# andrewcharlesjones/spatial-alignment

Hardware: AMD Instinct MI355X
Metric: training steps/sec (ELBO fwd+bwd), 2-view N=10k M=200, 1/2/4/8 GPU (higher is better)
Workload: dtype f32 (fp64 warp layer, covariance whitening and M x M factorisations)

## Files before the change

### include/gpsa_hip.h

```cpp
#ifndef GPSA_HIP_H
#define GPSA_HIP_H

#ifdef __cplusplus
extern "C" {
#endif

enum {
  GPSA_F32 = 0,
  GPSA_F64 = 1,
  GPSA_F32_X64 = 2,
  GPSA_F32_OUT64 = 3,
  GPSA_F32_ACC64 = 4
};
enum { GPSA_K_RBF = 0, GPSA_K_MATERN12 = 1, GPSA_K_MATERN32 = 2 };
enum { GPSA_EINVAL = -1, GPSA_EWORKSPACE = -2, GPSA_EUNSUPPORTED = -3 };

int gpsa_version(void);
const char* gpsa_build_arch(void);
const char* gpsa_source_hash(void);

int gpsa_kmat(int dtype, int in_dtype, int kind, const void* Z, int M, const void* X, long long C,
              int D, const void* ls_u, const void* var_u, double jitter, void* K, void* stream);

long long gpsa_kmat_bwd_workspace(int dtype, int M, long long C, int D);
// ... 65 lines not shown
                              const float* meanT, const double* q, const float* var_u, const float* eps, const float* Y,
                              long long N, int S, const float* noise_u, float* g, float* dmeanT, float* abar, double* part,
                              float* FT, void* workspace, long long workspace_bytes, void* stream);
int gpsa_quadform_elbo_delta_x3_f32(int omega_dtype, const float* alpha, const void* Omega, int M, long long C, int L,
                                    const float* delta, const double* q, const float* var_u, const float* eps,
                                    const float* Y, long long N, int S, const float* noise_u, float* g, float* dmeanT,
                                    float* abar, double* part, float* FT, void* workspace, long long workspace_bytes,
                                    void* stream);
int gpsa_quadform_elbo_skip_f32(int omega_dtype, const float* alpha, const void* Omega, int M, long long C, int L,
                                const float* meanT, const double* q, const float* var_u, const float* eps, const float* Y,
                                long long N, int S, const float* noise_u, float* g, float* dmeanT, float* abar,
                                double* part, float* FT, void* workspace, long long workspace_bytes, void* stream);
int gpsa_quadform_elbo_delta_skip_f32(int omega_dtype, const float* alpha, const void* Omega, int M, long long C, int L,
                                      const float* delta, const double* q, const float* var_u, const float* eps,
                                      const float* Y, long long N, int S, const float* noise_u, float* g, float* dmeanT,
                                      float* abar, double* part, float* FT, void* workspace, long long workspace_bytes,
                                      void* stream);
int gpsa_quadform_bwd_omega(int dtype, int out_dtype, const void* alpha, const void* g, int M, long long C,
                            int L, void* dOmega, void* workspace, long long workspace_bytes, void* stream);
int gpsa_quadform_bwd_omega_takes_delta(int M, long long C);
int gpsa_quadform_bwd_omega_delta_f32(int out_dtype, const float* alpha, const float* g, const float* dmeanT, int M,
                                      long long C, int L, void* dOmega, float* ddelta, double dbeta, void* workspace,
                                      long long workspace_bytes, void* stream);
long long gpsa_quadform_bwd_omega_x3_workspace(int M, long long C, int L);
int gpsa_quadform_bwd_omega_x3(int dtype, int out_dtype, const void* alpha, const void* g, int M, long long C, int L,
                               void* dOmega, void* workspace, long long workspace_bytes, void* stream);
int gpsa_quadform_bwd_omega_delta_x3(int out_dtype, const float* alpha, const float* g, const float* dmeanT, int M,
                                     long long C, int L, void* dOmega, float* ddelta, double dbeta, void* workspace,
                                     long long workspace_bytes, void* stream);

long long gpsa_whiten_workspace(int M);
int gpsa_whiten_f64(const double* Kinv, int in_dtype, const void* Kuf, int M, long long C,
                    int alpha_dtype, void* alpha, double* q, void* workspace, long long workspace_bytes,
                    void* stream);

int gpsa_panel_mm(int dtype, int p_dtype, int transP, const void* P, const void* X, int M, long long C,
                  void* Y, void* colsq, void* workspace, long long workspace_bytes, void* stream);

int gpsa_col_axpy(int dtype, const void* Y, const void* X, const void* d, double s, int M,
                  long long C, void* out, void* stream);

int gpsa_data_sample_fwd(const float* meanT, const float* v, const double* q, const float* var_u,
                         const float* eps, long long C, int L, float* F, float* Sigma, void* stream);
int gpsa_data_sample_bwd(const float* dF, const float* eps, const float* Sigma, const float* var_u,
                         long long C, int L, float* g, float* dmeanT, float* qbar, int dvar_dtype, void* dvar_u,
                         void* workspace, long long workspace_bytes, void* stream);
// ... 507 lines not shown
```

### spatial_alignment_amd/_lib.py

```python
import ctypes as C
import os

_HERE = os.path.dirname(os.path.abspath(__file__))
LIB_PATH = os.path.join(_HERE, "libgpsa_hip.so")

_vp, _i, _ll, _d = C.c_void_p, C.c_int, C.c_longlong, C.c_double

SIGNATURES = {
    "gpsa_version": (_i, []),
    "gpsa_build_arch": (C.c_char_p, []),
    "gpsa_source_hash": (C.c_char_p, []),
    "gpsa_kmat": (_i, [_i, _i, _i, _vp, _i, _vp, _ll, _i, _vp, _vp, _d, _vp, _vp]),
    "gpsa_kmat_bwd_workspace": (_ll, [_i, _i, _ll, _i]),
    "gpsa_kmat_bwd": (_i, [_i, _i, _i, _vp, _i, _vp, _ll, _i, _vp, _vp, _vp, _i, _vp, _vp, _vp, _vp, _ll, _vp]),
    "gpsa_gemm_workspace": (_ll, [_i, _i, _i, _i, _i]),
    "gpsa_gemm": (_i, [_i, _i, _i, _i, _i, _ll, _d, _vp, _ll, _ll, _vp, _ll, _ll, _d, _vp, _ll, _ll,
                       _i, _i, _vp, _ll, _vp]),
    "gpsa_omega_fwd": (_i, [_vp, _i, _i, _d, _vp, _vp]),
    "gpsa_omega_bwd": (_i, [_vp, _vp, _i, _i, _i, _vp, _vp]),
    "gpsa_omega_fwd2": (_i, [_vp, _i, _vp, _vp, _i, _vp, _i, _d, _vp]),
    "gpsa_omega_bwd2": (_i, [_vp, _vp, _vp, _i, _vp, _vp, _vp, _i, _i, _i, _vp]),
    "gpsa_chol_f64": (_i, [_vp, _i, _i, _vp, _vp, _vp]),
    "gpsa_tri_inv_f64": (_i, [_vp, _vp, _i, _i, _vp]),
    "gpsa_chol_inv_f64": (_i, [_vp, _vp, _i, _i, _vp, _vp, _vp]),
    "gpsa_experiment_split_bf16_product": (_i, [_vp, _vp, _i, _ll, _i, _i, _vp, _vp]),
    "gpsa_experiment_split_bf16_rate": (_i, [_i, _i, _vp, _vp]),
    "gpsa_chol_inv_sel_f64": (_i, [_vp, _vp, _i, _i, _i, _i, _i, _vp, _vp, _vp]),
    "gpsa_chol_inv_blocked_workspace": (_ll, [_i, _i]),
    "gpsa_chol_inv_blocked_f64": (_i, [_vp, _vp, _i, _i, _vp, _vp, _vp, _ll, _vp]),
    "gpsa_quadform_workspace": (_ll, [_i, _i, _ll, _i]),
    "gpsa_quadform_fwd": (_i, [_i, _i, _vp, _vp, _i, _ll, _i, _vp, _vp, _ll, _vp]),
    "gpsa_quadform_bwd_alpha": (_i, [_i, _i, _vp, _vp, _vp, _i, _ll, _i, _vp, _vp, _ll, _vp]),
    "gpsa_quadform_fwd_keep": (_i, [_i, _vp, _vp, _i, _ll, _i, _vp, _vp, _vp, _vp, _vp]),
    "gpsa_quadform_bwd_alpha_kept": (_i, [_i, _vp, _vp, _i, _ll, _i, _vp, _vp, _vp, _vp]),
    "gpsa_quadform_bwd_omega": (_i, [_i, _i, _vp, _vp, _i, _ll, _i, _vp, _vp, _ll, _vp]),
    "gpsa_quadform_bwd_omega_takes_delta": (_i, [_i, _ll]),
    "gpsa_quadform_bwd_omega_delta_f32": (_i, [_i, _vp, _vp, _vp, _i, _ll, _i, _vp, _vp, _d, _vp, _ll, _vp]),
    "gpsa_quadform_bwd_omega_x3_workspace": (_ll, [_i, _ll, _i]),
    "gpsa_quadform_bwd_omega_x3": (_i, [_i, _i, _vp, _vp, _i, _ll, _i, _vp, _vp, _ll, _vp]),
    "gpsa_quadform_bwd_omega_delta_x3": (_i, [_i, _vp, _vp, _vp, _i, _ll, _i, _vp, _vp, _d, _vp, _ll, _vp]),
    "gpsa_whiten_workspace": (_ll, [_i]),
    "gpsa_whiten_f64": (_i, [_vp, _i, _vp, _i, _ll, _i, _vp, _vp, _vp, _ll, _vp]),
    "gpsa_panel_mm": (_i, [_i, _i, _i, _vp, _vp, _i, _ll, _vp, _vp, _vp, _ll, _vp]),
    "gpsa_col_axpy": (_i, [_i, _vp, _vp, _vp, _d, _i, _ll, _vp, _vp]),
    "gpsa_data_sample_fwd": (_i, [_vp, _vp, _vp, _vp, _vp, _ll, _i, _vp, _vp, _vp]),
    "gpsa_data_sample_bwd": (_i, [_vp, _vp, _vp, _vp, _ll, _i, _vp, _vp, _vp, _i, _vp, _vp, _ll, _vp]),
    "gpsa_warp_sample_fwd": (_i, [_vp, _vp, _vp, _vp, _vp, _vp, _vp, _vp, _ll, _i, _i, _vp, _vp, _vp, _vp, _vp]),
    "gpsa_warp_sample_bwd": (_i, [_vp, _vp, _vp, _vp, _vp, _vp, _ll, _i, _i, _vp, _vp, _vp, _vp, _vp, _vp, _vp,
                                  _ll, _vp]),
    "gpsa_mean_resid_fwd": (_i, [_vp, _vp, _vp, _vp, _i, _i, _d, _vp, _vp, _vp]),
    "gpsa_mean_resid_bwd": (_i, [_vp, _vp, _vp, _i, _i, _d, _vp, _vp, _vp, _vp, _vp]),
    "gpsa_loglik_fwd": (_i, [_vp, _vp, _vp, _i, _ll, _i, _vp, _vp, _ll, _vp]),
    "gpsa_loglik_bwd": (_i, [_vp, _vp, _vp, _vp, _i, _ll, _i, _vp, _vp, _vp, _ll, _vp]),
    "gpsa_bdot": (_i, [_i, _vp, _ll, _vp, _ll, _ll, _i, _vp, _vp, _ll, _vp]),
    "gpsa_add_diag": (_i, [_i, _vp, _i, _i, _d, _vp]),
    "gpsa_mvn_kl_fwd": (_i, [_vp, _vp, _vp, _ll, _vp, _ll, _vp, _vp, _i, _i, _vp, _vp]),
    "gpsa_mvn_kl_bwd": (_i, [_vp, _vp, _vp, _ll, _vp, _ll, _vp, _vp, _vp, _i, _i, _vp, _vp, _vp, _vp]),
    "gpsa_mvn_kl_grouped_fwd": (_i, [_vp, _vp, _vp, _vp, _vp, _vp, _i, _i, _vp, _vp, _vp]),
    "gpsa_mvn_kl_grouped_bwd": (_i, [_vp, _vp, _vp, _vp, _vp, _vp, _vp, _vp, _vp, _i, _i, _i, _vp, _vp, _vp,
# ... 325 lines not shown
```

### spatial_alignment_amd/csrc/qf_common.hpp

```cpp
#pragma once
#include <stdlib.h>

#include "common.hpp"

namespace gpsa {

typedef float f32x4_t __attribute__((ext_vector_type(4)));

typedef float f32x4 __attribute__((ext_vector_type(4)));
typedef float f32x2 __attribute__((ext_vector_type(2)));

enum { MODE_QUAD = 0, MODE_ACCUM = 1, MODE_STORE = 2 };

enum { PACK_SYM_UPPER = 1, PACK_KSTEP = 2, PACK_KSTEP_LAST = 4 };

typedef __attribute__((address_space(3))) void* lds_ptr_t;

__device__ __forceinline__ void glds16(const float* gsrc, unsigned lds_base) {
  unsigned keep;
  asm volatile(
      "s_mov_b32 %0, m0\n\ts_mov_b32 m0, %2\n\ts_nop 0\n\tglobal_load_lds_dwordx4 %1, off\n\ts_mov_b32 m0, %0"
      : "=&s"(keep)
      : "v"(gsrc), "s"(lds_base)
      : "memory");
// ... 330 lines not shown
    for (int r = MB - 1; r >= 0; --r) {
      int best = -1;
      for (int w = 0; w < 4 && best < 0; ++w)
        if (cnt[w] + r + 1 <= cap) best = w;
      if (best < 0) {
        best = 0;
        for (int w = 1; w < 4; ++w)
          if (cnt[w] < cnt[best]) best = w;
      }
      for (int c = 0; c <= r; ++c) {
        rr[best][cnt[best]] = r;
        cc[best][cnt[best]] = c;
        ++cnt[best];
      }
    }
  }
  constexpr int max_cnt() const {
    int m = 0;
    for (int w = 0; w < 4; ++w) m = cnt[w] > m ? cnt[w] : m;
    return m;
  }
};

#define GPSA_GRAM_SHAPES(X) X(2, 2) X(4, 2) X(7, 2) X(13, 2) X(2, 1) X(4, 1) X(7, 1) X(13, 1) X(16, 1)
#define GPSA_GRAM_EXTERN(MB, NL)                                                \
  extern template __global__ void gram_mfma_kernel<MB, true, NL> GPSA_GRAM_SIG; \
  extern template __global__ void gram_mfma_kernel<MB, false, NL> GPSA_GRAM_SIG;
#define GPSA_GRAM_DEFINE(MB, NL)                                         \
  template __global__ void gram_mfma_kernel<MB, true, NL> GPSA_GRAM_SIG; \
  template __global__ void gram_mfma_kernel<MB, false, NL> GPSA_GRAM_SIG;
GPSA_GRAM_SHAPES(GPSA_GRAM_EXTERN)
constexpr int gram_max_nl(int mb) {
  GPSA_GRAM_SHAPES(GPSA_SHAPE_SECOND)
  return 0;
}
template <typename TO>
__global__ void gram_reduce_kernel(const float* __restrict__ part, int M, int MP, int L, int nsplit, TO* __restrict__ out,
                                   float* __restrict__ ddelta, float dbeta);
extern template __global__ void gram_reduce_kernel<float>(const float* __restrict__, int, int, int, int, float* __restrict__, float* __restrict__, float);
extern template __global__ void gram_reduce_kernel<double>(const float* __restrict__, int, int, int, int, double* __restrict__, float* __restrict__, float);

template <int MB>
__global__ void __launch_bounds__(256, 1) gram_x3_kernel(const unsigned short* __restrict__ img, const float* __restrict__ g,
                                                         const float* __restrict__ dmean, int M, long long C, int L,
                                                         int nsplit, float* __restrict__ part);
#define GPSA_GRAM_X3_SHAPES(X) X(2) X(4) X(7) X(13) X(16)
// ... 9 lines not shown
```

### spatial_alignment_amd/csrc/qf_gram.hip

```cpp
#include "qf_common.hpp"

namespace gpsa {

__device__ __attribute__((aligned(16))) const float gram_zero16[4] = {0.f, 0.f, 0.f, 0.f};


constexpr int GR_G = 4;

template <int MB, int NKB, int W, int NS, int NL, typename STG>
__device__ __forceinline__ void gram_wave_chunk(const float* __restrict__ img,
                                                const float* __restrict__ gvec, int kq,
                                                f32x4 (&acc)[NL][NS + GR_G], STG&& stage, int drow, int lane15) {
  constexpr GramPlan<MB> P{};
  constexpr int N = P.cnt[W];
  constexpr int NGRP = (((NS + GR_G - 1) / GR_G) + 1) & ~1;
  constexpr int NPW_ = (MB * NKB + 3) / 4;
  static_assert(NKB == 4, "one K block per staging wave");
  auto frag = [&](int kb, int tile_row) {
    return *reinterpret_cast<const float4*>(img + kb * (NPW_ * 256) + tile_row * 256);
  };
  auto tile_of = [](int s) { return s < N ? s : N - 1; };
  auto new_row = [&](int s) { return s < N && (s == 0 || P.rr[W][s] != P.rr[W][s - 1]); };
  float4 araw[2][GR_G], fb[2][GR_G];
  float4 gk[NL], gn[NL], arow[NL];
#pragma unroll
  for (int q = 0; q < NL; ++q) {
    gn[q] = gk[q] = *reinterpret_cast<const float4*>(gvec + q * GR_KC + kq * 4);
    arow[q] = make_float4(0.f, 0.f, 0.f, 0.f);
  }
  constexpr bool OWNS_LAST = [] {
    constexpr GramPlan<MB> Q{};
    for (int s = 0; s < Q.cnt[W]; ++s)
      if (Q.rr[W][s] == MB - 1) return true;
    return false;
  }();
  const bool dsel = OWNS_LAST && drow >= 0 && lane15 == drow;
  float4 dk[OWNS_LAST ? NL : 1], dn[OWNS_LAST ? NL : 1];
  if (OWNS_LAST) {
#pragma unroll
    for (int q = 0; q < NL; ++q)
      dn[q] = dk[q] = drow >= 0 ? *reinterpret_cast<const float4*>(gvec + (NL + q) * GR_KC + kq * 4)
                                : make_float4(0.f, 0.f, 0.f, 0.f);
  }
#define GPSA_GR_FETCH(SLOT, KB, GP)                                                           \
  _Pragma("unroll") for (int u = 0; u < GR_G; ++u) {                                          \
    const int t__ = tile_of(GR_G * (GP) + u);                                                 \
    if (new_row(GR_G * (GP) + u)) araw[SLOT][u] = frag(KB, P.rr[W][t__]);                     \
    fb[SLOT][u] = frag(KB, P.cc[W][t__]);                                                     \
  }
  GPSA_GR_FETCH(0, 0, 0)
#pragma unroll 1
  for (int kb = 0; kb < NKB; ++kb) {
#pragma unroll
    for (int q = 0; q < NL; ++q) gk[q] = gn[q];
    if (OWNS_LAST) {
#pragma unroll
      for (int q = 0; q < NL; ++q) dk[q] = dn[q];
    }
#pragma unroll
    for (int gp = 0; gp < NGRP; ++gp) {
      const int cur = gp & 1, nxt = cur ^ 1;
      if (gp + 1 < NGRP) {
        GPSA_GR_FETCH(nxt, kb, gp + 1)
      } else if (kb + 1 < NKB) {
#pragma unroll
        for (int q = 0; q < NL; ++q)
          gn[q] = *reinterpret_cast<const float4*>(gvec + q * GR_KC + (kb + 1) * 16 + kq * 4);
        if (OWNS_LAST && drow >= 0) {
#pragma unroll
          for (int q = 0; q < NL; ++q)
            dn[q] = *reinterpret_cast<const float4*>(gvec + (NL + q) * GR_KC + (kb + 1) * 16 + kq * 4);
        }
        GPSA_GR_FETCH(nxt, kb + 1, 0)
      }
      __builtin_amdgcn_sched_barrier(0);
      if (gp < 5) stage(kb, gp);
      __builtin_amdgcn_sched_barrier(0);
      float4 a[NL][GR_G];
      int sl[GR_G];
#pragma unroll
      for (int u = 0; u < GR_G; ++u) {
        const int s_ = GR_G * gp + u;
        sl[u] = s_ < N ? s_ : NS + u;
#pragma unroll
        for (int q = 0; q < NL; ++q) {
          if (new_row(s_)) {
            const float4 r_ = araw[cur][u];
            arow[q] = make_float4(r_.x * gk[q].x, r_.y * gk[q].y, r_.z * gk[q].z, r_.w * gk[q].w);
            if (OWNS_LAST && P.rr[W][s_ < N ? s_ : N - 1] == MB - 1 && drow >= 0) {
              const float4 d_ = dk[q];
              arow[q] = make_float4(dsel ? d_.x : arow[q].x, dsel ? d_.y : arow[q].y, dsel ? d_.z : arow[q].z,
                                    dsel ? d_.w : arow[q].w);
            }
          }
          a[q][u] = arow[q];
        }
      }
#define GPSA_GR_MMA(F)                                                                          \
  _Pragma("unroll") for (int q = 0; q < NL; ++q)                                                \
    _Pragma("unroll") for (int u = 0; u < GR_G; ++u)                                            \
      if (GR_G * gp + u < N)                                                                    \
        acc[q][sl[u]] = __builtin_amdgcn_mfma_f32_16x16x4f32(a[q][u].F, fb[cur][u].F, acc[q][sl[u]], 0, 0, 0);
      GPSA_GR_MMA(x)
      GPSA_GR_MMA(y)
      GPSA_GR_MMA(z)
      GPSA_GR_MMA(w)
#undef GPSA_GR_MMA
      __builtin_amdgcn_sched_barrier(0);
    }
  }
#undef GPSA_GR_FETCH
}

template <int MB, int W, int NS>
__device__ __forceinline__ void gram_wave_store(const f32x4 (&acc)[NS + GR_G], float* __restrict__ P_, int j,
                                                int kq) {
  constexpr GramPlan<MB> P{};
  constexpr int MP = MB * 16;
#pragma unroll
  for (int s = 0; s < P.cnt[W]; ++s)
#pragma unroll
    for (int r = 0; r < 4; ++r)
      P_[(long long)(P.rr[W][s] * 16 + kq * 4 + r) * MP + P.cc[W][s] * 16 + j] = acc[s][r];
}

template <int MB, bool ALIGNED, int NL, int W>
__device__ __forceinline__ void gram_wave_run(const float* __restrict__ alpha, const float* __restrict__ g,
                                              long long gstride, int M, long long C, int L, int nsplit, float* __restrict__ part,
                                              float* __restrict__ sA_, float* __restrict__ sG_,
                                              const float* __restrict__ dmean) {
  constexpr int MP = MB * 16;
  constexpr GramPlan<MB> PLAN{};
  constexpr int NS = PLAN.max_cnt();
  constexpr int NKB = GR_KC / 16, NPIECE = MB * NKB;
  constexpr int NPW = (NPIECE + 3) / 4;
  constexpr int SA_STRIDE = NPW * 4 * 256, SG_STRIDE = 2 * NL * GR_KC;
  const int nstage = (dmean != nullptr ? 2 : 1) * NL * (GR_KC / 4);
  const int drow = dmean != nullptr ? M - 16 * (MB - 1) : -1;
  const int tid = threadIdx.x, lane = tid & 63;
  constexpr int w = W;
  const int j = lane & 15, kq = lane >> 4;
  const int l0 = blockIdx.x * NL, sp = blockIdx.y;
  const long long nch = (C + GR_KC - 1) / GR_KC;
  const long long ch0 = (long long)sp * nch / nsplit, ch1 = (long long)(sp + 1) * nch / nsplit;

  f32x4 acc[NL][NS + GR_G];
#pragma unroll
  for (int q = 0; q < NL; ++q)
#pragma unroll
    for (int s = 0; s < NS + GR_G; ++s) acc[q][s] = (f32x4){0.f, 0.f, 0.f, 0.f};

  auto gsrc = [&](int ln, long long col) -> const float* {
    const int which = ln / (NL * (GR_KC / 4)), lq = min(l0 + (ln / (GR_KC / 4)) % NL, L - 1);
    if (which == 1) return col >= C ? gram_zero16 : dmean + (long long)lq * C + col;
    return (gstride == C && col >= C) ? gram_zero16 : g + (long long)lq * gstride + col;
  };
#define GPSA_GR_STAGE(CH, BUF)                                                               \
  {                                                                                          \
    const long long cb__ = (long long)(CH) * GR_KC;                                          \
    if (ALIGNED) {                                                                           \
       \
      long long col = cb__ + w * 16 + kq * 4;                                                \
      col = col < C - 4 ? col : C - 4;                                                       \
      _Pragma("unroll") for (int pc = 0; pc < NPW; ++pc) {                                   \
        if ((pc & 3) == 0)                                                                   \
          dma_set_m0(__builtin_amdgcn_readfirstlane(lds_addr(sA_ + (BUF) * SA_STRIDE + (w * NPW + pc) * 256))); \
        int row = (pc < MB ? pc : 0) * 16 + j;                                               \
        row = row < M ? row : M - 1;                                                         \
        const float* gp__ = alpha + (long long)row * C + col;                                \
        if ((pc & 3) == 0) glds16_m0<0>(gp__);                                               \
        if ((pc & 3) == 1) glds16_m0<1024>(gp__ - 256);                                      \
        if ((pc & 3) == 2) glds16_m0<2048>(gp__ - 512);                                      \
        if ((pc & 3) == 3) glds16_m0<3072>(gp__ - 768);                                      \
      }                                                                                      \
      if (lane < nstage) {                                                                   \
        dma_set_m0(__builtin_amdgcn_readfirstlane(lds_addr(sG_ + (BUF) * SG_STRIDE)));       \
        glds16_m0<0>(gsrc(lane, cb__ + (lane % (GR_KC / 4)) * 4));                           \
      }                                                                                      \
    } else {                                                                                 \
      for (int e = tid; e < NPIECE * 256; e += 256) {                                        \
        const int piece = e >> 8, ln = (e >> 2) & 63, r = e & 3;                             \
        const int rb = piece / NKB, kb = piece % NKB;                                        \
        const int row = rb * 16 + (ln & 15);                                                 \
        const long long col = cb__ + kb * 16 + (ln >> 4) * 4 + r;                            \
        sA_[(BUF) * SA_STRIDE + (kb * NPW + rb) * 256 + (e & 255)] =                         \
            (row < M && col < C) ? alpha[(long long)row * C + col] : 0.f;                    \
      }                                                                                      \
      if (tid < NL * GR_KC)           \
        sG_[(BUF) * SG_STRIDE + tid] = g[(long long)min(l0 + tid / GR_KC, L - 1) * gstride + cb__ + tid % GR_KC]; \
    }                                                                                        \
  }

  if (ch1 > ch0) GPSA_GR_STAGE(ch0, 0)
  GPSA_DMA_DRAIN();
  __syncthreads();
  int buf = 0;
  for (long long ch = ch0; ch < ch1; ++ch) {
    const bool more = ch + 1 < ch1;
    constexpr int NGRP_ = (((NS + GR_G - 1) / GR_G) + 1) & ~1;
    constexpr bool SPREAD = ALIGNED && NGRP_ >= 5;
    if (more && !SPREAD) GPSA_GR_STAGE(ch + 1, buf ^ 1)
    const float* img = sA_ + buf * SA_STRIDE + lane * 4;
    long long ncol = (ch + 1) * GR_KC + w * 16 + kq * 4;
    ncol = ncol < C - 4 ? ncol : C - 4;
    const float* nsrc = alpha + ncol;
    float* nimg = sA_ + (buf ^ 1) * SA_STRIDE + w * NPW * 256;
    auto stage = [&](int kb, int gp) {
      if (!SPREAD || !more) return;
      if (gp < 4) {
        const int pc = kb * 4 + gp;
        if (pc < NPW) {
          if (gp == 0) dma_set_m0(__builtin_amdgcn_readfirstlane(lds_addr(nimg + kb * 4 * 256)));
          int row = pc * 16 + j;
          row = row < M ? row : M - 1;
          const float* gp__ = nsrc + (long long)row * C;
          if (gp == 0) glds16_m0<0>(gp__);
          if (gp == 1) glds16_m0<1024>(gp__ - 256);
          if (gp == 2) glds16_m0<2048>(gp__ - 512);
          if (gp == 3) glds16_m0<3072>(gp__ - 768);
        }
      } else if (kb == 0 && lane < nstage) {
        dma_set_m0(__builtin_amdgcn_readfirstlane(lds_addr(sG_ + (buf ^ 1) * SG_STRIDE)));
        glds16_m0<0>(gsrc(lane, (ch + 1) * GR_KC + (lane % (GR_KC / 4)) * 4));
      }
    };
    static_assert(NPW <= 16, "four pieces per K block of the chunk being multiplied");
    gram_wave_chunk<MB, NKB, W, NS, NL>(img, sG_ + buf * SG_STRIDE, kq, acc, stage, drow, lane & 15);
    GPSA_DMA_DRAIN();
    __syncthreads();
    buf ^= 1;
  }
  GPSA_DMA_DRAIN();
#undef GPSA_GR_STAGE
#pragma unroll
  for (int q = 0; q < NL; ++q) {
    if (l0 + q >= L) break;
    float* P = part + ((long long)(l0 + q) * nsplit + sp) * MP * MP;
    gram_wave_store<MB, W, NS>(acc[q], P, j, kq);
  }
}

template <int MB, bool ALIGNED, int NL>
__global__ void __launch_bounds__(256, (MB >= 13 || NL > 1) ? 1 : 2)
gram_mfma_kernel(const float* __restrict__ alpha, const float* __restrict__ g, long long gstride, int M,
                 long long C, int L, int nsplit, float* __restrict__ part, const float* __restrict__ dmean) {
  constexpr int NKB = GR_KC / 16, NPIECE = MB * NKB;
  constexpr int NPW = (NPIECE + 3) / 4;
  __shared__ __attribute__((aligned(16))) float sA[2][NPW * 4 * 256];
  __shared__ __attribute__((aligned(16))) float sG[2][2 * NL * GR_KC];
  const int w = __builtin_amdgcn_readfirstlane(threadIdx.x >> 6);
  switch (w) {
    case 0: gram_wave_run<MB, ALIGNED, NL, 0>(alpha, g, gstride, M, C, L, nsplit, part, &sA[0][0], &sG[0][0], dmean); break;
    case 1: gram_wave_run<MB, ALIGNED, NL, 1>(alpha, g, gstride, M, C, L, nsplit, part, &sA[0][0], &sG[0][0], dmean); break;
    case 2: gram_wave_run<MB, ALIGNED, NL, 2>(alpha, g, gstride, M, C, L, nsplit, part, &sA[0][0], &sG[0][0], dmean); break;
    default: gram_wave_run<MB, ALIGNED, NL, 3>(alpha, g, gstride, M, C, L, nsplit, part, &sA[0][0], &sG[0][0], dmean); break;
  }
}

template <typename TO>
__global__ void gram_reduce_kernel(const float* __restrict__ part, int M, int MP, int L, int nsplit,
                                   TO* __restrict__ out, float* __restrict__ ddelta, float dbeta) {
  const int jj = blockIdx.x * 32 + (threadIdx.x & 31);
  const int i = blockIdx.y * 8 + (threadIdx.x >> 5);
  const int l = blockIdx.z;
  if (ddelta != nullptr && i == M && jj < M) {
    const float* p = part + (long long)l * nsplit * MP * MP + (long long)M * MP + jj;
    const long long mm = (long long)MP * MP;
    double s = 0.0;
    for (int sp = 0; sp < nsplit; ++sp) s += (double)p[sp * mm];
    float* d = ddelta + (long long)jj * L + l;
    *d = dbeta != 0.f ? dbeta * *d + (float)s : (float)s;
    return;
  }
  if (i >= M || jj > i) return;
  const float* p = part + (long long)l * nsplit * MP * MP + (long long)i * MP + jj;
  const long long mm = (long long)MP * MP;
  TO s = TO(0), s1 = TO(0), s2 = TO(0), s3 = TO(0);
  int sp = 0;
  for (; sp + 3 < nsplit; sp += 4) {
    s += (TO)p[sp * mm];
// ... 18 lines not shown
```

### spatial_alignment_amd/csrc/quadform.hip

```cpp
#include <stdlib.h>

#include "qf_common.hpp"

namespace gpsa {

template <typename T>
int gemm_launch(int transA, int transB, int m, int n, long long k, double alpha, const T* A,
                long long lda, long long sA, const T* B, long long ldb, long long sB, double beta,
                T* C, long long ldc, long long sC, int batch, int splitk, void* ws,
                long long ws_bytes, hipStream_t st);
template <typename T>
int gemm_launch_tri(int transA, int transB, int m, int n, long long k, double alpha, const T* A,
                    long long lda, long long sA, const T* B, long long ldb, long long sB, double beta,
                    T* C, long long ldc, long long sC, int batch, int splitk, void* ws,
                    long long ws_bytes, hipStream_t st, int tri);

template <typename T>
int gemm_launch_scaled(int transA, int transB, int m, int n, long long k, double alpha, const T* A,
                       long long lda, long long sA, const T* B, long long ldb, long long sB, double beta,
                       T* C, long long ldc, long long sC, int batch, int splitk, void* ws,
                       long long ws_bytes, hipStream_t st, int tri, const T* kscale, long long sKs,
                       const T* cscale, long long sCs);

template <typename TS, typename TD>
// ... 708 lines not shown
    return {pk, slack, pk + slab_floats(num_cus(), MB, elbo_x3_nct_for(MB)) * 4 + slack};
  }
  const long long pk = packed_bytes(MB, L);
  return {pk, 0, pk + slab_floats(2LL * num_cus(), MB, elbo_nct_for(MB)) * 4};
}

struct GramWs {
  int nl, nsplit;
  long long part;
  long long total;
};
static inline long long gram_gpad_floats(long long C, int L) { return (long long)L * cdiv(C, GR_KC) * GR_KC; }
static inline GramWs gram_ws(int MB, long long C, int L) {
  const int nl = gram_nl(MB, L, C), ns = gram_nsplit(C, (L + nl - 1) / nl, GR_KC);
  const long long part = ((gram_gpad_floats(C, L) + 63) / 64) * 64 * 4;
  return {nl, ns, part, part + (long long)L * ns * MB * 16 * MB * 16 * 4};
}
static inline GramWs gram_x3_ws(int MB, long long C, int L) {
  const int ns = gram_nsplit(C, L, 32);
  const long long part = cdiv(C, 32) * MB * 3 * 1024;
  return {1, ns, part, part + (long long)L * ns * MB * 16 * MB * 16 * 4};
}

static int gram_reduce_launch(const float* part, int M, int MB, int L, int ns, void* dOmega, int out_dtype, float* ddelta,
                              float dbeta, hipStream_t st) {
  dim3 rgrid((unsigned)cdiv(M, 32), (unsigned)cdiv(M + (ddelta != nullptr ? 1 : 0), 8), (unsigned)L);
  if (out_dtype == GPSA_F64)
    gram_reduce_kernel<double><<<rgrid, 256, 0, st>>>(part, M, MB * 16, L, ns, (double*)dOmega, ddelta, dbeta);
  else
    gram_reduce_kernel<float><<<rgrid, 256, 0, st>>>(part, M, MB * 16, L, ns, (float*)dOmega, ddelta, dbeta);
  GPSA_LAUNCH_CHECK();
  return 0;
}

static int gram_mfma_launch(int MBsel, const float* alpha, const float* g, int M, long long C, int L,
                            void* dOmega, int out_dtype, void* workspace, long long workspace_bytes, hipStream_t st,
                            const float* dmean = nullptr, float* ddelta = nullptr, float dbeta = 0.f) {
  const GramWs lay = gram_ws(MBsel, C, L);
  if (workspace_bytes < lay.total) return GPSA_EWORKSPACE;
  const int ns = lay.nsplit;
  const long long Cpad = cdiv(C, GR_KC) * GR_KC;
  float* ws = (float*)workspace;
  const float* gpad = ws;
  long long gstride = Cpad;
  float* part = (float*)((char*)workspace + lay.part);
  const bool al = (C % 4 == 0) && (C >= 8) && ((reinterpret_cast<uintptr_t>(alpha) & 15) == 0);
  if (dmean != nullptr && !(al && ((reinterpret_cast<uintptr_t>(g) | reinterpret_cast<uintptr_t>(dmean)) & 15) == 0))
    return GPSA_EUNSUPPORTED;
  if (al && (reinterpret_cast<uintptr_t>(g) & 15) == 0) {
    gpad = g;
    gstride = C;
  } else {
    pad_rows_kernel<<<(unsigned)cdiv((long long)L * Cpad, 256), 256, 0, st>>>(g, L, C, Cpad, ws);
    GPSA_LAUNCH_CHECK();
  }
  dim3 grid((unsigned)((L + lay.nl - 1) / lay.nl), (unsigned)ns);
#define GPSA_GRAM_CASE(MBV, NLV)                                                                                      \
  case MBV * 8 + NLV:                                                                                                 \
    if (al) gram_mfma_kernel<MBV, true, NLV><<<grid, 256, 0, st>>>(alpha, gpad, gstride, M, C, L, ns, part, dmean);   \
    else gram_mfma_kernel<MBV, false, NLV><<<grid, 256, 0, st>>>(alpha, gpad, gstride, M, C, L, ns, part, nullptr);   \
    break;
  switch (MBsel * 8 + lay.nl) {
    GPSA_GRAM_SHAPES(GPSA_GRAM_CASE)
    default:
      return GPSA_EUNSUPPORTED;
  }
#undef GPSA_GRAM_CASE
  GPSA_LAUNCH_CHECK();
  return gram_reduce_launch(part, M, MBsel, L, ns, dOmega, out_dtype, ddelta, dbeta, st);
}

template <typename TS, typename TD>
__global__ void convert_kernel(const TS* __restrict__ src, long long n, TD* __restrict__ dst) {
  const long long i = blockIdx.x * 256LL + threadIdx.x;
  if (i < n) dst[i] = (TD)src[i];
}

template <typename T>
static int operand_as(int p_dtype, const void* P, long long n, const T** out, void** ws,
                      long long* ws_bytes, hipStream_t st) {
// ... 590 lines not shown
        pad_cols_kernel<<<(unsigned)cdiv((long long)L * Cp, 256), 256, 0, st>>>((const float*)g, L, C, Cp, gp);
        GPSA_LAUNCH_CHECK();
        return generic_quadform_bwd_omega<float>(ap, gp, M, Cp, L, (float*)dOmega, workspace, rest, st);
      }
    }
    return generic_quadform_bwd_omega<float>((const float*)alpha, (const float*)g, M, C, L,
                                             (float*)dOmega, workspace, workspace_bytes, st);
  }
  if (dtype == GPSA_F64) {
    if (out_dtype != dtype) return GPSA_EUNSUPPORTED;
    return generic_quadform_bwd_omega<double>((const double*)alpha, (const double*)g, M, C, L,
                                              (double*)dOmega, workspace, workspace_bytes, st);
  }
  return GPSA_EINVAL;
}

static inline bool gram_delta_ok(int M, long long C) {
  const int MB = gpsa::gram_mb_for(M);
  return MB != 0 && !gpsa::force_generic() && gpsa::has_padding_row(M, MB) && (C % 4 == 0) && C >= 8;
}

int gpsa_quadform_bwd_omega_takes_delta(int M, long long C) { return M >= 1 && C >= 1 && gram_delta_ok(M, C) ? 1 : 0; }

int gpsa_quadform_bwd_omega_delta_f32(int out_dtype, const float* alpha, const float* g, const float* dmeanT, int M,
                                      long long C, int L, void* dOmega, float* ddelta, double dbeta, void* workspace,
                                      long long workspace_bytes, void* stream) {
  using namespace gpsa;
  if (M < 1 || C < 1 || L < 1 || !alpha || !g || !dmeanT || !dOmega || !ddelta) return GPSA_EINVAL;
  if (out_dtype != GPSA_F32 && out_dtype != GPSA_F64) return GPSA_EINVAL;
  if (!gram_delta_ok(M, C)) return GPSA_EUNSUPPORTED;
  return gram_mfma_launch(gram_mb_for(M), alpha, g, M, C, L, dOmega, out_dtype, workspace, workspace_bytes, as_stream(stream),
                          dmeanT, ddelta, (float)dbeta);
}

long long gpsa_quadform_bwd_omega_x3_workspace(int M, long long C, int L) {
  using namespace gpsa;
  if (M < 1 || C < 1 || L < 1 || L > 65535) return 0;
  const int MB = gram_mb_for(M);
  if (!MB || force_generic()) return 0;
  return gram_x3_ws(MB, C, L).total;
}

static int gram_x3_launch(int out_dtype, const float* alpha, const float* g, const float* dmean, int M, long long C, int L,
                          void* dOmega, float* ddelta, float dbeta, void* workspace, long long workspace_bytes,
                          hipStream_t st) {
  using namespace gpsa;
// ... 153 lines not shown
```

Before: 151.0.

## Add paired-output Gram kernel sharing the half-filled last row tile, with spare-CU delta workgroups

For M=200 (13 row tiles, last tile holding only 8 rows), a new Gram kernel packs the two outputs' partial last-tile rows into one MFMA tile. The lower 8 lanes serve output 0 and the upper 8 serve output 1, which drops the redundant MMAs on padding rows and rebalances the tile deal across the four waves. The delta (dmean) row product moves out of the owning wave into extra spare workgroups launched on idle CUs, and these write the padding row of each partial. This adds complexity, a hand-written deal for MB=13 only, and a heuristic for the spare-workgroup count.

```diff
diff --git a/include/gpsa_hip.h b/include/gpsa_hip.h
--- a/include/gpsa_hip.h
+++ b/include/gpsa_hip.h
@@ -111,6 +111,8 @@
 int gpsa_quadform_bwd_omega_delta_f32(int out_dtype, const float* alpha, const float* g, const float* dmeanT, int M,
                                       long long C, int L, void* dOmega, float* ddelta, double dbeta, void* workspace,
                                       long long workspace_bytes, void* stream);
+int gpsa_quadform_bwd_omega_pairs(int M, long long C, int L);
+int gpsa_quadform_bwd_omega_delta_spare(int M, long long C, int L);
 long long gpsa_quadform_bwd_omega_x3_workspace(int M, long long C, int L);
 int gpsa_quadform_bwd_omega_x3(int dtype, int out_dtype, const void* alpha, const void* g, int M, long long C, int L,
                                void* dOmega, void* workspace, long long workspace_bytes, void* stream);
diff --git a/spatial_alignment_amd/_lib.py b/spatial_alignment_amd/_lib.py
--- a/spatial_alignment_amd/_lib.py
+++ b/spatial_alignment_amd/_lib.py
@@ -35,6 +35,8 @@
     "gpsa_quadform_bwd_alpha_kept": (_i, [_i, _vp, _vp, _i, _ll, _i, _vp, _vp, _vp, _vp]),
     "gpsa_quadform_bwd_omega": (_i, [_i, _i, _vp, _vp, _i, _ll, _i, _vp, _vp, _ll, _vp]),
     "gpsa_quadform_bwd_omega_takes_delta": (_i, [_i, _ll]),
+    "gpsa_quadform_bwd_omega_pairs": (_i, [_i, _ll, _i]),
+    "gpsa_quadform_bwd_omega_delta_spare": (_i, [_i, _ll, _i]),
     "gpsa_quadform_bwd_omega_delta_f32": (_i, [_i, _vp, _vp, _vp, _i, _ll, _i, _vp, _vp, _d, _vp, _ll, _vp]),
     "gpsa_quadform_bwd_omega_x3_workspace": (_ll, [_i, _ll, _i]),
     "gpsa_quadform_bwd_omega_x3": (_i, [_i, _i, _vp, _vp, _i, _ll, _i, _vp, _vp, _ll, _vp]),
diff --git a/spatial_alignment_amd/csrc/qf_common.hpp b/spatial_alignment_amd/csrc/qf_common.hpp
--- a/spatial_alignment_amd/csrc/qf_common.hpp
+++ b/spatial_alignment_amd/csrc/qf_common.hpp
@@ -376,6 +376,38 @@
   }
 };
 
+template <int MB>
+struct GramPairPlan {
+  static_assert(MB == 13, "the deal is written out for 13 row tiles");
+  static constexpr int NT = MB * (MB + 1) / 2;
+  int cnt[4];
+  int rr[4][NT], cc[4][NT];
+  constexpr GramPairPlan() : cnt{}, rr{}, cc{} {
+    const int deal[4][6] = {{11, 8, -1, -1, -1, -1}, {10, 9, -1, -1, -1, -1}, {7, 6, 5, -1, -1, -1}, {12, 4, 3, 2, 1, 0}};
+    for (int w = 0; w < 4; ++w)
+      for (int i = 0; i < 6 && deal[w][i] >= 0; ++i)
+        for (int c = 0; c <= deal[w][i]; ++c) {
+          rr[w][cnt[w]] = deal[w][i];
+          cc[w][cnt[w]] = c;
+          ++cnt[w];
+        }
+  }
+  constexpr int max_cnt() const {
+    int m = 0;
+    for (int w = 0; w < 4; ++w) m = cnt[w] > m ? cnt[w] : m;
+    return m;
+  }
+};
+template <int MB, bool PAIR>
+struct GramPlanOf { using type = GramPlan<MB>; };
+template <int MB>
+struct GramPlanOf<MB, true> { using type = GramPairPlan<MB>; };
+constexpr bool gram_pair_rows(int M, int MB) { return M - 16 * (MB - 1) >= 1 && M - 16 * (MB - 1) <= 8; }
+constexpr int GR_SPARE_MAX = 64;
+template <int MB>
+__global__ void __launch_bounds__(256, 1) gram_pair_kernel(const float* __restrict__ alpha, const float* __restrict__ g, long long gstride, int M, long long C, int L, int nsplit, float* __restrict__ part, const float* __restrict__ dmean, int nspare);
+extern template __global__ void gram_pair_kernel<13>(const float* __restrict__, const float* __restrict__, long long, int, long long, int, int, float* __restrict__, const float* __restrict__, int);
+
 #define GPSA_GRAM_SHAPES(X) X(2, 2) X(4, 2) X(7, 2) X(13, 2) X(2, 1) X(4, 1) X(7, 1) X(13, 1) X(16, 1)
 #define GPSA_GRAM_EXTERN(MB, NL)                                                \
   extern template __global__ void gram_mfma_kernel<MB, true, NL> GPSA_GRAM_SIG; \
diff --git a/spatial_alignment_amd/csrc/qf_gram.hip b/spatial_alignment_amd/csrc/qf_gram.hip
--- a/spatial_alignment_amd/csrc/qf_gram.hip
+++ b/spatial_alignment_amd/csrc/qf_gram.hip
@@ -7,13 +7,19 @@
 
 constexpr int GR_G = 4;
 
-template <int MB, int NKB, int W, int NS, int NL, typename STG>
+constexpr int gram_ngrp(int n) { return (((n + GR_G - 1) / GR_G) + 1) & ~1; }
+constexpr int gram_pair_ngrp(int n) { return (n + GR_G - 1) / GR_G; }
+
+template <int MB, int NKB, int W, int NS, int NL, bool PAIR, typename STG>
 __device__ __forceinline__ void gram_wave_chunk(const float* __restrict__ img,
                                                 const float* __restrict__ gvec, int kq,
                                                 f32x4 (&acc)[NL][NS + GR_G], STG&& stage, int drow, int lane15) {
-  constexpr GramPlan<MB> P{};
+  constexpr typename GramPlanOf<MB, PAIR>::type P{};
   constexpr int N = P.cnt[W];
-  constexpr int NGRP = (((NS + GR_G - 1) / GR_G) + 1) & ~1;
+  constexpr int NGRP = PAIR ? gram_pair_ngrp(N) : gram_ngrp(NS);
+  constexpr int KBU = (NGRP & 1) ? 2 : 1;
+  static_assert(NKB % KBU == 0, "whole trips");
+  static_assert(!PAIR || NL == 2, "the paired last tile row is for two outputs");
   constexpr int NPW_ = (MB * NKB + 3) / 4;
   static_assert(NKB == 4, "one K block per staging wave");
   auto frag = [&](int kb, int tile_row) {
@@ -21,6 +27,7 @@
   };
   auto tile_of = [](int s) { return s < N ? s : N - 1; };
   auto new_row = [&](int s) { return s < N && (s == 0 || P.rr[W][s] != P.rr[W][s - 1]); };
+  auto shared_row = [&](int s) { return PAIR && s < N && P.rr[W][s] == MB - 1; };
   float4 araw[2][GR_G], fb[2][GR_G];
   float4 gk[NL], gn[NL], arow[NL];
 #pragma unroll
@@ -29,11 +36,13 @@
     arow[q] = make_float4(0.f, 0.f, 0.f, 0.f);
   }
   constexpr bool OWNS_LAST = [] {
-    constexpr GramPlan<MB> Q{};
+    if (PAIR) return false;
+    constexpr typename GramPlanOf<MB, PAIR>::type Q{};
     for (int s = 0; s < Q.cnt[W]; ++s)
       if (Q.rr[W][s] == MB - 1) return true;
     return false;
   }();
+  const bool hi = PAIR && lane15 >= 8;
   const bool dsel = OWNS_LAST && drow >= 0 && lane15 == drow;
   float4 dk[OWNS_LAST ? NL : 1], dn[OWNS_LAST ? NL : 1];
   if (OWNS_LAST) {
@@ -46,11 +55,14 @@
   _Pragma("unroll") for (int u = 0; u < GR_G; ++u) {                                          \
     const int t__ = tile_of(GR_G * (GP) + u);                                                 \
     if (new_row(GR_G * (GP) + u)) araw[SLOT][u] = frag(KB, P.rr[W][t__]);                     \
-    fb[SLOT][u] = frag(KB, P.cc[W][t__]);                                                     \
+    if (!PAIR || GR_G * (GP) + u < N) fb[SLOT][u] = frag(KB, P.cc[W][t__]);                   \
   }
   GPSA_GR_FETCH(0, 0, 0)
 #pragma unroll 1
-  for (int kb = 0; kb < NKB; ++kb) {
+  for (int kb0 = 0; kb0 < NKB; kb0 += KBU)
+#pragma unroll
+  for (int kbi = 0; kbi < KBU; ++kbi) {
+    const int kb = kb0 + kbi;
 #pragma unroll
     for (int q = 0; q < NL; ++q) gk[q] = gn[q];
     if (OWNS_LAST) {
@@ -59,7 +71,7 @@
     }
 #pragma unroll
     for (int gp = 0; gp < NGRP; ++gp) {
-      const int cur = gp & 1, nxt = cur ^ 1;
+      const int cur = (kbi * NGRP + gp) & 1, nxt = cur ^ 1;
       if (gp + 1 < NGRP) {
         GPSA_GR_FETCH(nxt, kb, gp + 1)
       } else if (kb + 1 < NKB) {
@@ -84,7 +96,13 @@
         sl[u] = s_ < N ? s_ : NS + u;
 #pragma unroll
         for (int q = 0; q < NL; ++q) {
-          if (new_row(s_)) {
+          if (new_row(s_) && shared_row(s_)) {
+            if (q == 0) {
+              const float4 r_ = araw[cur][u];
+              arow[0] = make_float4(r_.x * (hi ? gk[1].x : gk[0].x), r_.y * (hi ? gk[1].y : gk[0].y),
+                                    r_.z * (hi ? gk[1].z : gk[0].z), r_.w * (hi ? gk[1].w : gk[0].w));
+            }
+          } else if (new_row(s_)) {
             const float4 r_ = araw[cur][u];
             arow[q] = make_float4(r_.x * gk[q].x, r_.y * gk[q].y, r_.z * gk[q].z, r_.w * gk[q].w);
             if (OWNS_LAST && P.rr[W][s_ < N ? s_ : N - 1] == MB - 1 && drow >= 0) {
@@ -99,7 +117,7 @@
 #define GPSA_GR_MMA(F)                                                                          \
   _Pragma("unroll") for (int q = 0; q < NL; ++q)                                                \
     _Pragma("unroll") for (int u = 0; u < GR_G; ++u)                                            \
-      if (GR_G * gp + u < N)                                                                    \
+      if (GR_G * gp + u < N && (q == 0 || !shared_row(GR_G * gp + u)))                          \
         acc[q][sl[u]] = __builtin_amdgcn_mfma_f32_16x16x4f32(a[q][u].F, fb[cur][u].F, acc[q][sl[u]], 0, 0, 0);
       GPSA_GR_MMA(x)
       GPSA_GR_MMA(y)
@@ -124,14 +142,40 @@
       P_[(long long)(P.rr[W][s] * 16 + kq * 4 + r) * MP + P.cc[W][s] * 16 + j] = acc[s][r];
 }
 
-template <int MB, bool ALIGNED, int NL, int W>
+template <int MB, int W, int NS>
+__device__ __forceinline__ void gram_pair_store(const f32x4 (&acc)[2][NS + GR_G], float* __restrict__ P0,
+                                                float* __restrict__ P1, int M, int j, int kq) {
+  constexpr GramPairPlan<MB> P{};
+  constexpr int MP = MB * 16;
+#pragma unroll
+  for (int s = 0; s < P.cnt[W]; ++s) {
+    if (P.rr[W][s] == MB - 1) {
+      float* Ph = kq < 2 ? P0 : P1;
+#pragma unroll
+      for (int r = 0; r < 4; ++r) {
+        const int row = 16 * (MB - 1) + (kq & 1) * 4 + r;
+        if (Ph != nullptr && row < M) Ph[(long long)row * MP + P.cc[W][s] * 16 + j] = acc[0][s][r];
+      }
+    } else {
+#pragma unroll
+      for (int r = 0; r < 4; ++r) {
+        const long long at = (long long)(P.rr[W][s] * 16 + kq * 4 + r) * MP + P.cc[W][s] * 16 + j;
+        P0[at] = acc[0][s][r];
+        if (P1 != nullptr) P1[at] = acc[1][s][r];
+      }
+    }
+  }
+}
+
+template <int MB, bool ALIGNED, int NL, int W, bool PAIR = false>
 __device__ __forceinline__ void gram_wave_run(const float* __restrict__ alpha, const float* __restrict__ g,
                                               long long gstride, int M, long long C, int L, int nsplit, float* __restrict__ part,
                                               float* __restrict__ sA_, float* __restrict__ sG_,
-                                              const float* __restrict__ dmean) {
+                                              const float* __restrict__ dmean, int grp, int sp, bool zero_row = false) {
   constexpr int MP = MB * 16;
-  constexpr GramPlan<MB> PLAN{};
+  constexpr typename GramPlanOf<MB, PAIR>::type PLAN{};
   constexpr int NS = PLAN.max_cnt();
+  static_assert(!PAIR || (ALIGNED && NL == 2), "the paired form: aligned operands, two outputs");
   constexpr int NKB = GR_KC / 16, NPIECE = MB * NKB;
   constexpr int NPW = (NPIECE + 3) / 4;
   constexpr int SA_STRIDE = NPW * 4 * 256, SG_STRIDE = 2 * NL * GR_KC;
@@ -140,7 +184,7 @@
   const int tid = threadIdx.x, lane = tid & 63;
   constexpr int w = W;
   const int j = lane & 15, kq = lane >> 4;
-  const int l0 = blockIdx.x * NL, sp = blockIdx.y;
+  const int l0 = grp * NL;
   const long long nch = (C + GR_KC - 1) / GR_KC;
   const long long ch0 = (long long)sp * nch / nsplit, ch1 = (long long)(sp + 1) * nch / nsplit;
 
@@ -165,7 +209,7 @@
       _Pragma("unroll") for (int pc = 0; pc < NPW; ++pc) {                                   \
         if ((pc & 3) == 0)                                                                   \
           dma_set_m0(__builtin_amdgcn_readfirstlane(lds_addr(sA_ + (BUF) * SA_STRIDE + (w * NPW + pc) * 256))); \
-        int row = (pc < MB ? pc : 0) * 16 + j;                                               \
+        int row = (pc < MB ? pc : 0) * 16 + (PAIR && pc == MB - 1 ? (j & 7) : j);            \
         row = row < M ? row : M - 1;                                                         \
         const float* gp__ = alpha + (long long)row * C + col;                                \
         if ((pc & 3) == 0) glds16_m0<0>(gp__);                                               \
@@ -197,7 +241,7 @@
   int buf = 0;
   for (long long ch = ch0; ch < ch1; ++ch) {
     const bool more = ch + 1 < ch1;
-    constexpr int NGRP_ = (((NS + GR_G - 1) / GR_G) + 1) & ~1;
+    constexpr int NGRP_ = PAIR ? gram_pair_ngrp(PLAN.cnt[W]) : gram_ngrp(NS);
     constexpr bool SPREAD = ALIGNED && NGRP_ >= 5;
     if (more && !SPREAD) GPSA_GR_STAGE(ch + 1, buf ^ 1)
     const float* img = sA_ + buf * SA_STRIDE + lane * 4;
@@ -211,7 +255,7 @@
         const int pc = kb * 4 + gp;
         if (pc < NPW) {
           if (gp == 0) dma_set_m0(__builtin_amdgcn_readfirstlane(lds_addr(nimg + kb * 4 * 256)));
-          int row = pc * 16 + j;
+          int row = pc * 16 + (PAIR && pc == MB - 1 ? (j & 7) : j);
           row = row < M ? row : M - 1;
           const float* gp__ = nsrc + (long long)row * C;
           if (gp == 0) glds16_m0<0>(gp__);
@@ -225,18 +269,30 @@
       }
     };
     static_assert(NPW <= 16, "four pieces per K block of the chunk being multiplied");
-    gram_wave_chunk<MB, NKB, W, NS, NL>(img, sG_ + buf * SG_STRIDE, kq, acc, stage, drow, lane & 15);
+    gram_wave_chunk<MB, NKB, W, NS, NL, PAIR>(img, sG_ + buf * SG_STRIDE, kq, acc, stage, drow, lane & 15);
     GPSA_DMA_DRAIN();
     __syncthreads();
     buf ^= 1;
   }
   GPSA_DMA_DRAIN();
 #undef GPSA_GR_STAGE
-#pragma unroll
-  for (int q = 0; q < NL; ++q) {
-    if (l0 + q >= L) break;
-    float* P = part + ((long long)(l0 + q) * nsplit + sp) * MP * MP;
-    gram_wave_store<MB, W, NS>(acc[q], P, j, kq);
+  if constexpr (PAIR) {
+    float* P0 = part + ((long long)l0 * nsplit + sp) * MP * MP;
+    float* P1 = l0 + 1 < L ? part + ((long long)(l0 + 1) * nsplit + sp) * MP * MP : nullptr;
+    gram_pair_store<MB, W, NS>(acc, P0, P1, M, j, kq);
+    if (W == 3 && zero_row) {
+      for (int c = lane; c < MP; c += 64) {
+        P0[(long long)M * MP + c] = 0.f;
+        if (P1 != nullptr) P1[(long long)M * MP + c] = 0.f;
+      }
+    }
+  } else {
+#pragma unroll
+    for (int q = 0; q < NL; ++q) {
+      if (l0 + q >= L) break;
+      float* P = part + ((long long)(l0 + q) * nsplit + sp) * MP * MP;
+      gram_wave_store<MB, W, NS>(acc[q], P, j, kq);
+    }
   }
 }
 
@@ -250,12 +306,100 @@
   __shared__ __attribute__((aligned(16))) float sG[2][2 * NL * GR_KC];
   const int w = __builtin_amdgcn_readfirstlane(threadIdx.x >> 6);
   switch (w) {
-    case 0: gram_wave_run<MB, ALIGNED, NL, 0>(alpha, g, gstride, M, C, L, nsplit, part, &sA[0][0], &sG[0][0], dmean); break;
-    case 1: gram_wave_run<MB, ALIGNED, NL, 1>(alpha, g, gstride, M, C, L, nsplit, part, &sA[0][0], &sG[0][0], dmean); break;
-    case 2: gram_wave_run<MB, ALIGNED, NL, 2>(alpha, g, gstride, M, C, L, nsplit, part, &sA[0][0], &sG[0][0], dmean); break;
-    default: gram_wave_run<MB, ALIGNED, NL, 3>(alpha, g, gstride, M, C, L, nsplit, part, &sA[0][0], &sG[0][0], dmean); break;
-  }
-}
+    case 0: gram_wave_run<MB, ALIGNED, NL, 0>(alpha, g, gstride, M, C, L, nsplit, part, &sA[0][0], &sG[0][0], dmean, blockIdx.x, blockIdx.y); break;
+    case 1: gram_wave_run<MB, ALIGNED, NL, 1>(alpha, g, gstride, M, C, L, nsplit, part, &sA[0][0], &sG[0][0], dmean, blockIdx.x, blockIdx.y); break;
+    case 2: gram_wave_run<MB, ALIGNED, NL, 2>(alpha, g, gstride, M, C, L, nsplit, part, &sA[0][0], &sG[0][0], dmean, blockIdx.x, blockIdx.y); break;
+    default: gram_wave_run<MB, ALIGNED, NL, 3>(alpha, g, gstride, M, C, L, nsplit, part, &sA[0][0], &sG[0][0], dmean, blockIdx.x, blockIdx.y); break;
+  }
+}
+
+
+constexpr int GR_SPARE_AHEAD = 3;
+
+template <int MB>
+__device__ __forceinline__ void gram_spare_run(const float* __restrict__ alpha, const float* __restrict__ dmean, int M,
+                                               long long C, int L, int nsplit, float* __restrict__ part, int k, int nspare) {
+  constexpr int MP = MB * 16, RING = GR_SPARE_AHEAD + 1;
+  const int lane = threadIdx.x & 63, w = threadIdx.x >> 6, j = lane & 15, kq = lane >> 4;
+  const long long nkb = (C + 15) / 16;
+  const long long kb0 = (long long)k * nkb / nspare, kb1 = (long long)(k + 1) * nkb / nspare;
+  if (kb1 <= kb0) {
+    for (int e = threadIdx.x; e < L * MP; e += 256)
+      part[((long long)(e / MP) * nsplit + k) * MP * MP + (long long)M * MP + e % MP] = 0.f;
+    return;
+  }
+  const float* arow[MB];
+#pragma unroll
+  for (int rt = 0; rt < MB; ++rt) arow[rt] = alpha + (long long)min(16 * rt + j, M - 1) * C + kq * 4;
+  for (int ot = w; ot * 16 < L; ot += 4) {
+    const float* drow = dmean + (long long)min(16 * ot + j, L - 1) * C + kq * 4;
+    f32x4 acc[MB];
+#pragma unroll
+    for (int rt = 0; rt < MB; ++rt) acc[rt] = (f32x4){0.f, 0.f, 0.f, 0.f};
+    float4 fa[RING], fb[RING][MB];
+    auto load = [&](long long kb, float4& a, float4 (&b)[MB]) {
+      kb = kb < kb1 ? kb : kb1 - 1;
+      long long col = kb * 16;
+      col = col + kq * 4 < C ? col : C - 4 - kq * 4;
+      a = *reinterpret_cast<const float4*>(drow + col);
+#pragma unroll
+      for (int rt = 0; rt < MB; ++rt) b[rt] = *reinterpret_cast<const float4*>(arow[rt] + col);
+    };
+#pragma unroll
+    for (int d = 0; d < GR_SPARE_AHEAD; ++d) load(kb0 + d, fa[d], fb[d]);
+    for (long long kb = kb0; kb < kb1; kb += RING) {
+#pragma unroll
+      for (int d = 0; d < RING; ++d) {
+        load(kb + d + GR_SPARE_AHEAD, fa[(d + GR_SPARE_AHEAD) % RING], fb[(d + GR_SPARE_AHEAD) % RING]);
+        __builtin_amdgcn_sched_barrier(0);
+        const bool in = kb + d < kb1 && (kb + d) * 16 + kq * 4 < C;
+        const float4 a_ = make_float4(in ? fa[d].x : 0.f, in ? fa[d].y : 0.f, in ? fa[d].z : 0.f, in ? fa[d].w : 0.f);
+#define GPSA_SPARE_MMA(F)                         \
+  _Pragma("unroll") for (int rt = 0; rt < MB; ++rt) \
+    acc[rt] = __builtin_amdgcn_mfma_f32_16x16x4f32(a_.F, fb[d][rt].F, acc[rt], 0, 0, 0);
+        GPSA_SPARE_MMA(x)
+        GPSA_SPARE_MMA(y)
+        GPSA_SPARE_MMA(z)
+        GPSA_SPARE_MMA(w)
+#undef GPSA_SPARE_MMA
+        __builtin_amdgcn_sched_barrier(0);
+      }
+    }
+#pragma unroll
+    for (int r = 0; r < 4; ++r) {
+      const int l = 16 * ot + 4 * kq + r;
+      if (l >= L) continue;
+      float* row = part + ((long long)l * nsplit + k) * MP * MP + (long long)M * MP;
+#pragma unroll
+      for (int rt = 0; rt < MB; ++rt)
+        if (16 * rt + j < M) row[16 * rt + j] = acc[rt][r];
+    }
+  }
+}
+
+template <int MB>
+__global__ void __launch_bounds__(256, 1)
+gram_pair_kernel(const float* __restrict__ alpha, const float* __restrict__ g, long long gstride, int M, long long C,
+                 int L, int nsplit, float* __restrict__ part, const float* __restrict__ dmean, int nspare) {
+  constexpr int NKB = GR_KC / 16, NPW = (MB * NKB + 3) / 4;
+  __shared__ __attribute__((aligned(16))) float sA[2][NPW * 4 * 256];
+  __shared__ __attribute__((aligned(16))) float sG[2][2 * 2 * GR_KC];
+  const int groups = (L + 1) / 2, b = blockIdx.x;
+  if (b >= groups * nsplit) {
+    gram_spare_run<MB>(alpha, dmean, M, C, L, nsplit, part, b - groups * nsplit, nspare);
+    return;
+  }
+  const int grp = b % groups, sp = b / groups;
+  const bool zero_row = dmean != nullptr && sp >= nspare;
+  const int w = __builtin_amdgcn_readfirstlane(threadIdx.x >> 6);
+  switch (w) {
+    case 0: gram_wave_run<MB, true, 2, 0, true>(alpha, g, gstride, M, C, L, nsplit, part, &sA[0][0], &sG[0][0], nullptr, grp, sp, zero_row); break;
+    case 1: gram_wave_run<MB, true, 2, 1, true>(alpha, g, gstride, M, C, L, nsplit, part, &sA[0][0], &sG[0][0], nullptr, grp, sp, zero_row); break;
+    case 2: gram_wave_run<MB, true, 2, 2, true>(alpha, g, gstride, M, C, L, nsplit, part, &sA[0][0], &sG[0][0], nullptr, grp, sp, zero_row); break;
+    default: gram_wave_run<MB, true, 2, 3, true>(alpha, g, gstride, M, C, L, nsplit, part, &sA[0][0], &sG[0][0], nullptr, grp, sp, zero_row); break;
+  }
+}
+template __global__ void gram_pair_kernel<13>(const float* __restrict__, const float* __restrict__, long long, int, long long, int, int, float* __restrict__, const float* __restrict__, int);
 
 template <typename TO>
 __global__ void gram_reduce_kernel(const float* __restrict__ part, int M, int MP, int L, int nsplit,
diff --git a/spatial_alignment_amd/csrc/quadform.hip b/spatial_alignment_amd/csrc/quadform.hip
--- a/spatial_alignment_amd/csrc/quadform.hip
+++ b/spatial_alignment_amd/csrc/quadform.hip
@@ -754,6 +754,17 @@
   return {1, ns, part, part + (long long)L * ns * MB * 16 * MB * 16 * 4};
 }
 
+static inline bool gram_pairs(int MB, int M, long long C, int L) {
+  return MB == 13 && gram_nl(MB, L, C) == 2 && gram_pair_rows(M, MB) && C % 4 == 0 && C >= 8;
+}
+static inline int gram_spare_wgs(int MB, int L, int groups, int ns) {
+  long long n = (long long)num_cus() - (long long)groups * ns;
+  n = n < GR_SPARE_MAX ? n : GR_SPARE_MAX;
+  n = n < ns ? n : ns;
+  const long long spare = (long long)MB * cdiv(cdiv(L, 16), 4) * ns, gram = 43 * n;
+  return (n >= 1 && 3 * spare <= 2 * gram) ? (int)n : 0;
+}
+
 static int gram_reduce_launch(const float* part, int M, int MB, int L, int ns, void* dOmega, int out_dtype, float* ddelta,
                               float dbeta, hipStream_t st) {
   dim3 rgrid((unsigned)cdiv(M, 32), (unsigned)cdiv(M + (ddelta != nullptr ? 1 : 0), 8), (unsigned)L);
@@ -786,8 +797,17 @@
     pad_rows_kernel<<<(unsigned)cdiv((long long)L * Cpad, 256), 256, 0, st>>>(g, L, C, Cpad, ws);
     GPSA_LAUNCH_CHECK();
   }
+  if (al && gram_pairs(MBsel, M, C, L)) {
+    const int groups = (L + 1) / 2, nspare = dmean != nullptr ? gram_spare_wgs(MBsel, L, groups, ns) : 0;
+    if (dmean == nullptr || nspare > 0) {
+      gram_pair_kernel<13><<<dim3((unsigned)(groups * ns + nspare)), 256, 0, st>>>(alpha, gpad, gstride, M, C, L, ns, part,
+                                                                                  dmean, nspare);
+      GPSA_LAUNCH_CHECK();
+      return gram_reduce_launch(part, M, MBsel, L, ns, dOmega, out_dtype, ddelta, dbeta, st);
+    }
+  }
   dim3 grid((unsigned)((L + lay.nl - 1) / lay.nl), (unsigned)ns);
-#define GPSA_GRAM_CASE(MBV, NLV)                                                                                      \
+#define GPSA_GRAM_CASE(MBV, NLV)                                                                                     \
   case MBV * 8 + NLV:                                                                                                 \
     if (al) gram_mfma_kernel<MBV, true, NLV><<<grid, 256, 0, st>>>(alpha, gpad, gstride, M, C, L, ns, part, dmean);   \
     else gram_mfma_kernel<MBV, false, NLV><<<grid, 256, 0, st>>>(alpha, gpad, gstride, M, C, L, ns, part, nullptr);   \
@@ -1424,6 +1444,18 @@
 
 int gpsa_quadform_bwd_omega_takes_delta(int M, long long C) { return M >= 1 && C >= 1 && gram_delta_ok(M, C) ? 1 : 0; }
 
+int gpsa_quadform_bwd_omega_pairs(int M, long long C, int L) {
+  if (M < 1 || C < 1 || L < 1) return 0;
+  const int MB = gpsa::gram_mb_for(M);
+  return MB != 0 && !gpsa::force_generic() && gpsa::gram_pairs(MB, M, C, L) ? 1 : 0;
+}
+
+int gpsa_quadform_bwd_omega_delta_spare(int M, long long C, int L) {
+  if (!gpsa_quadform_bwd_omega_pairs(M, C, L)) return 0;
+  const int groups = (L + 1) / 2;
+  return gpsa::gram_spare_wgs(13, L, groups, gpsa::gram_nsplit(C, groups, gpsa::GR_KC));
+}
+
 int gpsa_quadform_bwd_omega_delta_f32(int out_dtype, const float* alpha, const float* g, const float* dmeanT, int M,
                                       long long C, int L, void* dOmega, float* ddelta, double dbeta, void* workspace,
                                       long long workspace_bytes, void* stream) {
```

After: 151.9, median of 6. No clear change (+0.6%).
